# trevor-m/cuda-pathtrace

Hardware: AMD Instinct MI355X
Metric: Msamples/s, 9-sphere Cornell box 1024x1024x1024spp (higher is better)
Workload: dtype f32+f64

## Files before the change

cuda-pathtrace_amd/csrc/pt_intersect.h:

```cpp
#pragma once
#include "pt_scene_lds.h"

#pragma clang fp contract(off)

namespace pt {

template <int LEVEL>
__device__ __forceinline__ bool intersect_scene_loop(const SceneLds& sc, int n, F3 o, F3 d, const RayConst& rc,
                                                     float& t_hit, int& idx) {
  float tNearest = 1000000.0f;
  float t = 0.0f;
  bool hit = false;
#pragma clang loop unroll(disable)
  for (int i = 0; i < n; i++) {
    const float4 g = sc.geom_uniform(i);
    bool h;
    if constexpr (LEVEL == 0)
      h = intersect_sphere(o, d, rc.a, g, t);
    else
      h = intersect_sphere_v1(o, d, rc, g, t);
    if (h && t > 0.0f && t < tNearest) {
      tNearest = t;
      hit = true;
      t_hit = t;
      idx = i;
    }
  }
  return hit;
}

__device__ __forceinline__ bool intersect_scene_screened(const SceneLds& sc, int n, F3 o, F3 d, const RayConst& rc,
                                                         float& t_hit, int& idx) {
  const float INF = __builtin_inff();
  const float Tlim = 1000000.0f * (2.0f * rc.a);
  const float Tlim_hi = Tlim * 1.0000153f;
  float T1 = INF, T2 = INF;
  int i1 = 0;
  bool unsure = false;
PT_UNROLL(PT_SCREEN_UNROLL)
  for (int i = 0; i < n; i++) {
    const float4 g = sc.geom[i];
    const F3 off = mk3(o.x - g.x, o.y - g.y, o.z - g.z);
    const float b = 2.0f * dot(d, off);
    const float c = dot(off, off) - g.w;
    const float bb = b * b;
    const float a4c = rc.a4 * c;
    const float det = bb - a4c;
    const float dacc = fmaf(-rc.a4, c, bb);
    const float s = __builtin_amdgcn_sqrtf(fmaxf(dacc, 0.0f));
    const float q = b + copysign_b3(s, b);
    const float TA = -q;
    const float e = fmaf(b, b, -bb);
    const float num = a4c + e;
    const float TB = -num * __builtin_amdgcn_rcpf(q);
    const float lo = fminf(TA, TB), hi = fmaxf(TA, TB);
    const float T = lo > 0.0f ? lo : hi;
    const bool real = det >= 0.0f && dacc >= 0.0f;
    const bool ok = real && T > 0.0f && T < Tlim_hi;
    unsure = unsure || (real && !(fabsf(num) > fabsf(a4c) * 4.7683716e-07f && fabsf(T) < INF));
    const float Te = ok ? T : INF;
    const bool c1 = Te < T1, c2 = Te < T2;
    T2 = c1 ? T1 : (c2 ? Te : T2);
    i1 = c1 ? i : i1;
    T1 = c1 ? Te : T1;
  }
  bool ambiguous = unsure || (T1 < INF && (T2 <= T1 * 1.0000038f || T1 >= Tlim * 0.99998f));
  bool hit = false;
  if (!ambiguous && T1 < INF) {
    float t;
    if (intersect_sphere_v1(o, d, rc, sc.geom[i1], t) && t > 0.0f && t < 1000000.0f) {
      hit = true;
      t_hit = t;
      idx = i1;
    } else {
      ambiguous = true;
    }
  }
  if (__builtin_expect(ambiguous, 0)) hit = intersect_scene_loop<1>(sc, n, o, d, rc, t_hit, idx);
  return hit;
}

__device__ __forceinline__ void screen_tail(float b, float a4c, float det, float dacc, float num, float TA, float TB,
                                            float Tlim_hi, int i, float& T1, float& T2, int& i1, bool& unsure) {
  const float INF = __builtin_inff();
  const float lo = fminf(TA, TB), hi = fmaxf(TA, TB);
  const float T = lo > 0.0f ? lo : hi;
  const bool real = (det >= 0.0f) & (dacc >= 0.0f);
  const bool ok = real & (T > 0.0f) & (T < Tlim_hi);
  unsure = unsure | (real & !((fabsf(num) > fabsf(a4c) * 4.7683716e-07f) & (fabsf(T) < INF)));
  const float Te = ok ? T : INF;
  const bool c1 = Te < T1, c2 = Te < T2;
  T2 = c1 ? T1 : (c2 ? Te : T2);
  i1 = c1 ? i : i1;
  T1 = c1 ? Te : T1;
  (void)b;
}

__device__ __forceinline__ bool intersect_scene_screened_pk(const SceneLds& sc, int n, F3 o, F3 d, const RayConst& rc,
                                                            float& t_hit, int& idx) {
  const float INF = __builtin_inff();
  const float Tlim = 1000000.0f * (2.0f * rc.a);
  const float Tlim_hi = Tlim * 1.0000153f;
  float T1 = INF, T2 = INF;
  int i1 = 0;
  bool unsure = false;
  const v2f ox = {o.x, o.x}, oy = {o.y, o.y}, oz = {o.z, o.z};
  const v2f dx = {d.x, d.x}, dy = {d.y, d.y}, dz = {d.z, d.z};
  const v2f a4 = {rc.a4, rc.a4};
  const int npairs = (n + 1) >> 1;
  for (int p = 0; p < npairs; p++) {
    const float4 A = sc.pair[2 * p], B = sc.pair[2 * p + 1];
    const v2f offx = ox - v2f{A.x, A.y}, offy = oy - v2f{A.z, A.w}, offz = oz - v2f{B.x, B.y};
    const v2f dd = dx * offx + dy * offy + dz * offz;
    const v2f b = dd + dd;
    const v2f c = (offx * offx + offy * offy + offz * offz) - v2f{B.z, B.w};
    const v2f bb = b * b;
    const v2f a4c = a4 * c;
    const v2f det = bb - a4c;
    const v2f dacc = __builtin_elementwise_fma(-a4, c, bb);
    const v2f e = __builtin_elementwise_fma(b, b, -bb);
    const v2f num = a4c + e;
    const v2f s = {__builtin_amdgcn_sqrtf(fmaxf(dacc.x, 0.0f)), __builtin_amdgcn_sqrtf(fmaxf(dacc.y, 0.0f))};
    const v2f q = b + v2f{copysignf(s.x, b.x), copysignf(s.y, b.y)};
    const v2f r = {__builtin_amdgcn_rcpf(q.x), __builtin_amdgcn_rcpf(q.y)};
    const v2f TA = -q;
    const v2f TB = -num * r;
    screen_tail(b.x, a4c.x, det.x, dacc.x, num.x, TA.x, TB.x, Tlim_hi, 2 * p, T1, T2, i1, unsure);
    screen_tail(b.y, a4c.y, det.y, dacc.y, num.y, TA.y, TB.y, Tlim_hi, 2 * p + 1, T1, T2, i1, unsure);
  }
  bool ambiguous = unsure | ((T1 < INF) & ((T2 <= T1 * 1.0000038f) | (T1 >= Tlim * 0.99998f)));
  bool hit = false;
  if (!ambiguous && T1 < INF) {
    float t;
    if (intersect_sphere_v1(o, d, rc, sc.geom[i1], t) && t > 0.0f && t < 1000000.0f) {
      hit = true;
      t_hit = t;
      idx = i1;
    } else {
      ambiguous = true;
    }
  }
  if (__builtin_expect(ambiguous, 0)) hit = intersect_scene_loop<1>(sc, n, o, d, rc, t_hit, idx);
  return hit;
}

__device__ __forceinline__ uint32_t umed3(uint32_t a, uint32_t b, uint32_t c) {
  uint32_t r;
  asm("v_med3_u32 %0, %1, %2, %3" : "=v"(r) : "v"(a), "v"(b), "v"(c));
  return r;
}

struct ScreenState {
  uint32_t k1, k2;
  bool unsure;
  uint32_t absmask;
};

__device__ __forceinline__ uint32_t screen_sphere_oc(F3 off, float c, int i, F3 d, const RayConst& rc, uint32_t imask, ScreenState& st);
__device__ __forceinline__ uint32_t screen_sphere(const float4 g, int i, F3 o, F3 d, const RayConst& rc, uint32_t imask,
                                                  ScreenState& st) {
  const F3 off = mk3(o.x - g.x, o.y - g.y, o.z - g.z);
  return screen_sphere_oc(off, dot(off, off) - g.w, i, d, rc, imask, st);
}
__device__ __forceinline__ void screen_insert(ScreenState& st, uint32_t key) {
  st.k2 = umed3(st.k1, st.k2, key);
  st.k1 = st.k1 < key ? st.k1 : key;
}
template <class F>
__device__ __forceinline__ void screen_nine(ScreenState& st, F key_of) {
  auto umin = [](uint32_t x, uint32_t y) { return x < y ? x : y; };
  auto umax = [](uint32_t x, uint32_t y) { return x > y ? x : y; };
  uint32_t lead[3], next[3];
#pragma unroll
  for (int g3 = 0; g3 < 3; g3++) {
    const uint32_t x = key_of(3 * g3), y = key_of(3 * g3 + 1), z = key_of(3 * g3 + 2);
    lead[g3] = umin(umin(x, y), z);
    next[g3] = umed3(x, y, z);
  }
  const uint32_t l = umin(lead[0], lead[1]);
  const uint32_t r2 = umin(umin(umax(lead[0], lead[1]), next[0]), next[1]);
  st.k1 = umin(l, lead[2]);
  st.k2 = umin(umin(umax(l, lead[2]), r2), next[2]);
}
__device__ __forceinline__ uint32_t screen_sphere_oc(F3 off, float c, int i, F3 d, const RayConst& rc, uint32_t imask, ScreenState& st) {
  const float h = dot(d, off);
  const float hh = h * h;
  const float ac = rc.a * c;
  const float dacc = fmaf(-rc.a, c, hh);
  const float s = __builtin_amdgcn_sqrtf(dacc);
  const float e = fmaf(h, h, -hh);
  const float num = ac + e;
  const float TA = copysign_neg_b3(s, h, st.absmask) - h;
  const float TB = num * __builtin_amdgcn_rcpf(TA);
  const uint32_t ta = __float_as_uint(TA), tb = __float_as_uint(TB);
  const uint32_t tbits = ta < tb ? ta : tb;
  const uint32_t key = bitop3<0xBA>(tbits, imask, (uint32_t)i);
#ifndef PT_MUTANT_NO_DOUBT
  st.unsure = st.unsure | !(fabsf(ac) > fmaf(hh, 1.1920929e-07f, 1e-30f));
#endif
  return key;
}

__device__ __forceinline__ bool neg_finite(float x) { return __builtin_amdgcn_classf(x, 0x18); }
template <int AX>
__device__ __forceinline__ F3 with_axis(F3 v, float x) {
  return mk3(AX == 0 ? x : v.x, AX == 1 ? x : v.y, AX == 2 ? x : v.z);
}
template <int AX>
__device__ __forceinline__ uint32_t screen_wall_pair(const uint4 t, uint32_t m, F3 o, F3 d, const RayConst& rc, uint32_t imask,
                                                     ScreenState& st, float& hb, bool& inb) {
  const float4 gf = lds_read_f4(bitop3<0xE4>(t.y, t.x, m)), gb = lds_read_f4(bitop3<0xE4>(t.x, t.y, m));
  const F3 off = mk3(o.x - gf.x, o.y - gf.y, o.z - gf.z);
  const F3 sq = off * off, pr = d * off;
  const float ob = AX == 0 ? o.x - gb.x : AX == 1 ? o.y - gb.y : o.z - gb.z;
  const F3 sqb = with_axis<AX>(sq, ob * ob), prb = with_axis<AX>(pr, (AX == 0 ? d.x : AX == 1 ? d.y : d.z) * ob);
  hb = (prb.x + prb.y) + prb.z;
  inb = neg_finite(fmaf(gb.w, 5.9837103e-08f, ((sqb.x + sqb.y) + sqb.z) - gb.w));
  return screen_sphere_oc(off, ((sq.x + sq.y) + sq.z) - gf.w, (int)bitop3<0xE4>(t.w, t.z, m), d, rc, imask, st);
}
template <bool WALLS>
__device__ __forceinline__ void screen_walled(ScreenState& st, const uint4* W, F3 o, F3 d, const RayConst& rc, uint32_t imask,
                                              uint32_t lim_hi_bits) {
  auto umin = [](uint32_t x, uint32_t y) { return x < y ? x : y; };
  auto umax = [](uint32_t x, uint32_t y) { return x > y ? x : y; };
  const float4* Wg = reinterpret_cast<const float4*>(W);
  const uint4 oi = W[3];
  auto sel = [](uint32_t dbits) { return (uint32_t)((int32_t)dbits >> 31); };
  const uint32_t mx = sel(__float_as_uint(d.x)), my = sel(__float_as_uint(d.y)), mz = sel(__float_as_uint(d.z));
  const uint32_t a0 = screen_sphere(Wg[0], (int)oi.x, o, d, rc, imask, st), a1 = screen_sphere(Wg[1], (int)oi.y, o, d, rc, imask, st),
                 a2 = screen_sphere(Wg[2], (int)oi.z, o, d, rc, imask, st);
  const uint32_t l0 = umin(umin(a0, a1), a2), n0 = umed3(a0, a1, a2);
  float h0, h1, h2;
  bool in0, in1, in2;
  if constexpr (WALLS) __builtin_amdgcn_sched_barrier(0);
  const uint32_t b0 = screen_wall_pair<0>(W[4], mx, o, d, rc, imask, st, h0, in0);
  if constexpr (WALLS) __builtin_amdgcn_sched_barrier(0);
  const uint32_t b1 = screen_wall_pair<1>(W[5], my, o, d, rc, imask, st, h1, in1);
  if constexpr (WALLS) __builtin_amdgcn_sched_barrier(0);
  const uint32_t b2 = screen_wall_pair<2>(W[6], mz, o, d, rc, imask, st, h2, in2);
  if constexpr (WALLS) __builtin_amdgcn_sched_barrier(0);
  const uint32_t l1 = umin(umin(b0, b1), b2), n1 = umed3(b0, b1, b2);
  st.k1 = umin(l0, l1);
  st.k2 = umin(umin(umax(l0, l1), n0), n1);
  const float K = __uint_as_float(st.k1 & ~imask) * __uint_as_float(oi.w);
  const bool cert = (st.k1 < lim_hi_bits) & (neg_finite(fmaf(2.0f, h0, K)) & in0) & (neg_finite(fmaf(2.0f, h1, K)) & in1) &
                    (neg_finite(fmaf(2.0f, h2, K)) & in2);
  if (__builtin_expect(__builtin_amdgcn_ballot_w64(!cert) != 0, 0)) {
    auto behind = [&](int k, uint32_t m) {
      const uint4 t = W[4 + k];
      screen_insert(st, screen_sphere(lds_read_f4(bitop3<0xE4>(t.x, t.y, m)), (int)bitop3<0xE4>(t.z, t.w, m), o, d, rc, imask, st));
    };
    behind(0, mx);
    behind(1, my);
    behind(2, mz);
  }
}

#ifdef PT_SCREEN_STATS
__device__ unsigned long long g_screen_stats[8];
#endif
template <bool NB, bool PRIMARY = false, bool LAST = false, bool WALLS = false>
__device__ __forceinline__ bool intersect_scene_screened_keys(const SceneLds& sc, int n, F3 o, F3 d, const RayConst& rc,
                                                              float& t_hit, int& idx) {
  if (n <= 0) return false;
  const float Tlim = 1000000.0f * rc.a;
  const uint32_t lim_hi_bits = __float_as_uint(Tlim * 1.0000153f);
  const int ib = 32 - __builtin_clz((unsigned)(n > 1 ? n - 1 : 1));
  const uint32_t imask = (1u << ib) - 1u;
  const float margin = 1.0f + (__builtin_ldexpf(1.0f, ib - 22) + 7.6293945e-06f);
  ScreenState st{0xFFFFFFFFu, 0xFFFFFFFFu, false, sc.absmask};
  auto key_of = [&](const float4 g, int i) -> uint32_t {
    if constexpr (PRIMARY) {
      const float4 e = sc.eyeg[i];
      return screen_sphere_oc(mk3(e.x, e.y, e.z), e.w, i, d, rc, imask, st);
    } else {
      return screen_sphere(g, i, o, d, rc, imask, st);
    }
  };
  auto screen = [&](const float4 g, int i) { screen_insert(st, key_of(g, i)); };
  int i = 0;
  if constexpr (PRIMARY) {
    const uint32_t full = n >= 32 ? 0xFFFFFFFFu : (1u << n) - 1u;
    uint32_t m = __builtin_amdgcn_readfirstlane(sc.prim_mask) & full;
    if (m != full) {
      while (m) {
        const int j = __builtin_ctz(m);
        m &= m - 1u;
        screen(sc.geom[j], j);
      }
      i = n;
    }
  }
#if PT_UNROLL_NINE
  if constexpr (!PRIMARY) {
    if (sc.walls && n == 9) {
      screen_walled<WALLS>(st, sc.walls, o, d, rc, imask, lim_hi_bits);
      i = 9;
    }
  }
  if (i == 0 && n == 9) {
    screen_nine(st, [&](int u) { return key_of(sc.geom[u], u); });
    i = 9;
  }
#endif
  for (; i + 3 <= n; i += 3) {
    const float4 g0 = sc.geom[i], g1 = sc.geom[i + 1], g2 = sc.geom[i + 2];
    screen(g0, i);
    screen(g1, i + 1);
    screen(g2, i + 2);
  }
  for (; i < n; i++) screen(sc.geom[i], i);
  const uint32_t k1 = st.k1, k2 = st.k2;
  const bool has = k1 < lim_hi_bits;
  const float T1 = __uint_as_float(k1 & ~imask);
  bool ambiguous = st.unsure | (has & (((k2 & ~imask) <= __float_as_uint(T1 * margin)) | (T1 >= Tlim * 0.99998f)));
  bool hit = false;
  if constexpr (NB && LAST && !PRIMARY) {
    const int i1 = (int)(k1 & imask);
    const float4 g = sc.geom[has ? i1 : 0];
    const F3 off = mk3(o.x - g.x, o.y - g.y, o.z - g.z);
    const float h = dot(d, off);
    const float c = dot(off, off) - g.w;
    const float ac = rc.a * c;
    const float dacc = fmaf(-rc.a, c, h * h);
    const bool certain = (dacc > fabsf(ac) * 4.7683716e-07f) & (T1 >= rc.a * 1e-30f);
    ambiguous = ambiguous | (has & !certain);
    hit = has;
    t_hit = T1;
    idx = i1;
    if (__builtin_expect(ambiguous, 0)) hit = intersect_scene_loop<0>(sc, n, o, d, rc, t_hit, idx);
    return hit;
  } else if constexpr (NB) {
    const int i1 = (int)(k1 & imask);
    float t;
    bool bad = false;
    bool real;
    if constexpr (PRIMARY) {
      const float4 e = sc.eyeg[has ? i1 : 0];
      real = intersect_sphere_nb_oc(mk3(e.x, e.y, e.z), e.w, d, rc, t, bad);
    } else {
      real = intersect_sphere_nb(o, d, rc, sc.geom[has ? i1 : 0], t, bad);
    }
    const bool good = real & (t >= kMinGoodT) & (t < 1000000.0f);
#ifdef PT_SCREEN_STATS
    {
      const bool tie = has & ((k2 & ~imask) <= __float_as_uint(T1 * margin));
      const bool lim = has & (T1 >= Tlim * 0.99998f);
      const uint64_t any = __builtin_amdgcn_ballot_w64(ambiguous | (has & (bad | !good)));
      if ((threadIdx.x & 63) == __builtin_ctzll(__builtin_amdgcn_ballot_w64(true))) {
        atomicAdd(&g_screen_stats[0], 1ull);
        atomicAdd(&g_screen_stats[1], any != 0 ? 1ull : 0ull);
      }
      atomicAdd(&g_screen_stats[2], (ambiguous | (has & (bad | !good))) ? 1ull : 0ull);
      atomicAdd(&g_screen_stats[3], st.unsure ? 1ull : 0ull);
      atomicAdd(&g_screen_stats[4], tie ? 1ull : 0ull);
      atomicAdd(&g_screen_stats[5], lim ? 1ull : 0ull);
      atomicAdd(&g_screen_stats[6], (has & bad) ? 1ull : 0ull);
      atomicAdd(&g_screen_stats[7], (has & !good) ? 1ull : 0ull);
    }
#endif
    ambiguous = ambiguous | (has & (bad | !good));
    hit = has & good;
    t_hit = t;
    idx = i1;
#ifdef PT_TIMING_ONLY_DETECT_NO_REDO
    if (__builtin_expect(ambiguous, 0)) hit = false;
#elif !defined(PT_TIMING_ONLY_NO_ISECT_REDO)
    if (__builtin_expect(ambiguous, 0)) hit = intersect_scene_loop<0>(sc, n, o, d, rc, t_hit, idx);
#endif
    return hit;
  } else {
    if (!ambiguous && has) {
      const int i1 = (int)(k1 & imask);
      float t;
      if (intersect_sphere_v1(o, d, rc, sc.geom[i1], t) && t > 0.0f && t < 1000000.0f) {
        hit = true;
        t_hit = t;
        idx = i1;
      } else {
        ambiguous = true;
      }
    }
    if (__builtin_expect(ambiguous, 0)) hit = intersect_scene_loop<1>(sc, n, o, d, rc, t_hit, idx);
    return hit;
  }
}

__device__ __forceinline__ bool intersect_scene_screened_large(const SceneLds& sc, int n, F3 o, F3 d, const RayConst& rc,
                                                               float& t_hit, int& idx) {
  if (n <= 0) return false;
  const float INF = __builtin_inff();
  const float Tlim = 1000000.0f * (2.0f * rc.a);
  const float Tlim_hi = Tlim * 1.0000153f;
  float T1 = INF, T2 = INF;
  int i1 = 0;
  bool unsure = false;
  struct Head {
    float b, a4c, bb, dacc;
  };
  auto head = [&](const float4 g) {
    const F3 off = mk3(o.x - g.x, o.y - g.y, o.z - g.z);
    Head h;
    h.b = 2.0f * dot(d, off);
    const float c = dot(off, off) - g.w;
    h.bb = h.b * h.b;
    h.a4c = rc.a4 * c;
    h.dacc = fmaf(-rc.a4, c, h.bb);
    return h;
  };
  auto tail = [&](const Head& h, int i) {
    const bool cand = (int)__float_as_uint(h.dacc) >= 0;
    if (__builtin_amdgcn_ballot_w64(cand) == 0) return;
    const float s = __builtin_amdgcn_sqrtf(h.dacc);
    const float e = fmaf(h.b, h.b, -h.bb);
    const float num = h.a4c + e;
    const float TA = copysign_neg_b3(s, h.b, sc.absmask) - h.b;
    const float TB = num * __builtin_amdgcn_rcpf(TA);
    const uint32_t ta = __float_as_uint(TA), tb = __float_as_uint(TB);
    const uint32_t tbits = ta < tb ? ta : tb;
    const float T = __uint_as_float(tbits);
    const bool ok = tbits < __float_as_uint(Tlim_hi);
    unsure = unsure | (cand & !(fabsf(h.a4c) > fmaf(h.bb, 1.1920929e-07f, 1e-30f)));
    const float Te = ok ? T : INF;
    const bool c1 = Te < T1, c2 = Te < T2;
    T2 = c1 ? T1 : (c2 ? Te : T2);
    i1 = c1 ? i : i1;
    T1 = c1 ? Te : T1;
  };
  int i = 0;
  auto four = [&](const float4 g0, const float4 g1, const float4 g2, const float4 g3) {
    const Head h0 = head(g0), h1 = head(g1), h2 = head(g2), h3 = head(g3);
    const uint32_t all = __float_as_uint(h0.dacc) & __float_as_uint(h1.dacc) & __float_as_uint(h2.dacc) & __float_as_uint(h3.dacc);
    if (__builtin_amdgcn_ballot_w64((int)all >= 0) != 0) {
      tail(h0, i);
      tail(h1, i + 1);
      tail(h2, i + 2);
      tail(h3, i + 3);
    }
  };
  if (sc.lean) {
    typedef uint32_t u4 __attribute__((ext_vector_type(4)));
    const pt_sphere* base = sc.global;
    auto request = [&](u4& dst, int k) {
      const uint32_t off = (uint32_t)(k < n ? k : n - 1) * (uint32_t)sizeof(pt_sphere);
      asm volatile("s_load_dwordx4 %[dst], %[base], %[off]" : [dst] "=s"(dst), "+v"(o.x) : [base] "s"(base), [off] "s"(off));
    };
    auto as_geom = [](const u4 v) {
      const float r = __uint_as_float(v.x);
      return make_float4(__uint_as_float(v.y), __uint_as_float(v.z), __uint_as_float(v.w), r * r);
    };
    if (n >= 4) {
      u4 a0, a1, a2, a3;
      request(a0, 0);
      request(a1, 1);
      request(a2, 2);
      request(a3, 3);
      asm volatile("s_waitcnt lgkmcnt(0)" : "+s"(a0), "+s"(a1), "+s"(a2), "+s"(a3));
      for (; i + 4 <= n; i += 4) {
        u4 b0, b1, b2, b3;
        request(b0, i + 4);
        request(b1, i + 5);
        request(b2, i + 6);
        request(b3, i + 7);
        four(as_geom(a0), as_geom(a1), as_geom(a2), as_geom(a3));
        asm volatile("s_waitcnt lgkmcnt(0)" : "+s"(b0), "+s"(b1), "+s"(b2), "+s"(b3));
        a0 = b0;
        a1 = b1;
        a2 = b2;
        a3 = b3;
      }
    }
  } else {
    for (; i + 4 <= n; i += 4) four(sc.geom[i], sc.geom[i + 1], sc.geom[i + 2], sc.geom[i + 3]);
  }
  for (; i < n; i++) tail(head(sc.geom_uniform(i)), i);
  const bool has = T1 < INF;
  bool ambiguous = unsure | (has & ((T2 <= T1 * 1.0000038f) | (T1 >= Tlim * 0.99998f)));
  float t;
  bool bad = false;
  const bool real = intersect_sphere_nb(o, d, rc, sc.geom_lane(i1), t, bad);
  const bool good = real & (t >= kMinGoodT) & (t < 1000000.0f);
  ambiguous = ambiguous | (has & (bad | !good));
  t_hit = t;
  idx = i1;
  bool hit = has & good;
  if (__builtin_expect(ambiguous, 0)) hit = intersect_scene_loop<0>(sc, n, o, d, rc, t_hit, idx);
  return hit;
}

template <int LEVEL, bool PRIMARY = false, bool LAST = false, bool WALLS = false>
__device__ __forceinline__ bool intersect_scene(const SceneLds& sc, int n, F3 o, F3 d, float& t_hit, int& idx) {
  const RayConst rc = (LEVEL >= 6 && !PRIMARY && !sc.lean) ? make_ray_const_unit(d, sc.rden1) : make_ray_const(d);
  if constexpr (LEVEL >= 5) {
    if (!sc.lean && (sc.small_only || n <= PT_SCREEN_MAX_SPHERES))
      return intersect_scene_screened_keys<(LEVEL >= 6), (PRIMARY && LEVEL >= 6), (LAST && LEVEL >= 6), WALLS>(sc, n, o, d, rc, t_hit, idx);
    if constexpr (LEVEL >= 6) return intersect_scene_screened_large(sc, n, o, d, rc, t_hit, idx);
    return intersect_scene_loop<1>(sc, n, o, d, rc, t_hit, idx);
  }
  if constexpr (LEVEL == 3)
    return intersect_scene_screened_pk(sc, n, o, d, rc, t_hit, idx);
  else if constexpr (LEVEL == 2 || LEVEL == 4)
    return intersect_scene_screened(sc, n, o, d, rc, t_hit, idx);
  else
    return intersect_scene_loop<LEVEL>(sc, n, o, d, rc, t_hit, idx);
}

template <int P, bool PRIMARY = false, bool LAST = false>
__device__ __forceinline__ void intersect_paths(const SceneLds& sc, int n, const F3 (&o)[P], const F3 (&d)[P],
                                                bool (&hit)[P], float (&t_hit)[P], int (&idx)[P]) {
  RayConst rc[P];
  ScreenState st[P];
#pragma unroll
  for (int p = 0; p < P; p++) {
    rc[p] = (!PRIMARY && !sc.lean) ? make_ray_const_unit(d[p], sc.rden1) : make_ray_const(d[p]);
    st[p] = ScreenState{0xFFFFFFFFu, 0xFFFFFFFFu, false, sc.absmask};
    hit[p] = false;
  }
  if (n <= 0) return;
  if (sc.lean || (!sc.small_only && n > PT_SCREEN_MAX_SPHERES)) {
#pragma unroll
    for (int p = 0; p < P; p++) hit[p] = intersect_scene_screened_large(sc, n, o[p], d[p], rc[p], t_hit[p], idx[p]);
    return;
  }
  const int ib = 32 - __builtin_clz((unsigned)(n > 1 ? n - 1 : 1));
  const uint32_t imask = (1u << ib) - 1u;
  const float margin = 1.0f + (__builtin_ldexpf(1.0f, ib - 22) + 7.6293945e-06f);
  int i = 0;
  if constexpr (PRIMARY && P == 1) {
    const uint32_t full = n >= 32 ? 0xFFFFFFFFu : (1u << n) - 1u;
    uint32_t m = __builtin_amdgcn_readfirstlane(sc.prim_mask) & full;
    if (n <= 16 && m != full) {
      while (m) {
        const int j = __builtin_ctz(m);
        m &= m - 1u;
        const float4 e = sc.eyeg[j];
        screen_insert(st[0], screen_sphere_oc(mk3(e.x, e.y, e.z), e.w, j, d[0], rc[0], imask, st[0]));
      }
      i = n;
    }
  }
#if PT_UNROLL_NINE
  if (i == 0 && P == 1 && n == 9) {
    screen_nine(st[0], [&](int u) -> uint32_t {
      if constexpr (PRIMARY) {
        const float4 e = sc.eyeg[u];
        return screen_sphere_oc(mk3(e.x, e.y, e.z), e.w, u, d[0], rc[0], imask, st[0]);
      } else {
        return screen_sphere(sc.geom[u], u, o[0], d[0], rc[0], imask, st[0]);
      }
    });
    i = 9;
  }
#endif
  for (; i + 2 <= n; i += 2) {
    const float4 g0 = sc.geom[i], g1 = sc.geom[i + 1];
#pragma unroll
    for (int p = 0; p < P; p++) {
      screen_insert(st[p], screen_sphere(g0, i, o[p], d[p], rc[p], imask, st[p]));
      screen_insert(st[p], screen_sphere(g1, i + 1, o[p], d[p], rc[p], imask, st[p]));
    }
  }
  for (; i < n; i++) {
    const float4 g = sc.geom[i];
#pragma unroll
    for (int p = 0; p < P; p++) screen_insert(st[p], screen_sphere(g, i, o[p], d[p], rc[p], imask, st[p]));
  }
  bool ambiguous[P];
#pragma unroll
  for (int p = 0; p < P; p++) {
    const float Tlim = 1000000.0f * rc[p].a;
    const bool has = st[p].k1 < __float_as_uint(Tlim * 1.0000153f);
    const float T1 = __uint_as_float(st[p].k1 & ~imask);
    ambiguous[p] = st[p].unsure | (has & (((st[p].k2 & ~imask) <= __float_as_uint(T1 * margin)) | (T1 >= Tlim * 0.99998f)));
    const int i1 = (int)(st[p].k1 & imask);
    if constexpr (LAST && !PRIMARY) {
      const float4 g = sc.geom[has ? i1 : 0];
      const F3 off = mk3(o[p].x - g.x, o[p].y - g.y, o[p].z - g.z);
      const float h = dot(d[p], off);
      const float c = dot(off, off) - g.w;
      const float dacc = fmaf(-rc[p].a, c, h * h);
      const bool certain = (dacc > fabsf(rc[p].a * c) * 4.7683716e-07f) & (T1 >= rc[p].a * 1e-30f);
      ambiguous[p] = ambiguous[p] | (has & !certain);
      hit[p] = has;
      t_hit[p] = T1;
      idx[p] = i1;
      continue;
    }
    float t;
    bool bad = false;
    bool real;
    if (PRIMARY && P == 1 && n <= 16) {
      const float4 e = sc.eyeg[has ? i1 : 0];
      real = intersect_sphere_nb_oc(mk3(e.x, e.y, e.z), e.w, d[p], rc[p], t, bad);
    } else {
      real = intersect_sphere_nb(o[p], d[p], rc[p], sc.geom[has ? i1 : 0], t, bad);
    }
    const bool good = real & (t >= kMinGoodT) & (t < 1000000.0f);
    ambiguous[p] = ambiguous[p] | (has & (bad | !good));
    hit[p] = has & good;
    t_hit[p] = t;
    idx[p] = i1;
  }
#pragma unroll
  for (int p = 0; p < P; p++)
    if (__builtin_expect(ambiguous[p], 0)) hit[p] = intersect_scene_loop<0>(sc, n, o[p], d[p], rc[p], t_hit[p], idx[p]);
}

}
```

cuda-pathtrace_amd/csrc/pt_scene_lds.h:

```cpp
#pragma once
#include "pt_device.h"
#include "pt_kernel.h"
#include "pt_walls.h"

#pragma clang fp contract(off)

namespace pt {

#define PT_PRAGMA_(x) _Pragma(#x)
#define PT_UNROLL(n) PT_PRAGMA_(unroll n)

struct GridLds;

struct SceneLds {
  float4* geom;
  float4* mat0;
  float4* mat1;
  float4* eyeg;
  float* inv1;
  double* rden1;
  float* rcpn;
  float4* pair;
  const pt_sphere* global;
  bool lean;
  bool small_only;
  const GridLds* grid;
  void* pool;
  uint32_t prim_mask;
  uint32_t absmask;
  const uint4* walls = nullptr;

  __device__ __forceinline__ float4 geom_uniform(int i) const {
    if (lean) {
      typedef float f4u __attribute__((ext_vector_type(4), aligned(4)));
      typedef const __attribute__((address_space(4))) f4u* cptr;
      typedef const __attribute__((address_space(4))) char* cbytes;
      const f4u v = *(cptr)((cbytes)global + (size_t)i * sizeof(pt_sphere));
      return make_float4(v.y, v.z, v.w, v.x * v.x);
    }
    return geom[i];
  }
  __device__ __forceinline__ float4 geom_lane(int i) const {
    if (lean) {
      const pt_sphere* sp = global + i;
      return make_float4(sp->pos[0], sp->pos[1], sp->pos[2], sp->radius * sp->radius);
    }
    return geom[i];
  }
};

typedef float v2f __attribute__((ext_vector_type(2)));

constexpr int kTablesF4 = kUnitTabSize / 4 + kUnitTabSize / 2 + (kRcpTab + 4) / 4;

template <bool WITH_PAIR>
__device__ __forceinline__ SceneLds stage_scene(const pt_sphere* __restrict__ spheres, int n, float4* lds, bool lean, F3 eye,
                                                int spp, bool lean_tables = true) {
  float4* tab = lean ? lds : lds + 4 * n;
  const bool tables = !lean | lean_tables;
  SceneLds s{lds, lds + n, lds + 2 * n, lds + 3 * n, tables ? reinterpret_cast<float*>(tab) : nullptr,
             tables ? reinterpret_cast<double*>(tab + kUnitTabSize / 4) : nullptr,
             tables ? reinterpret_cast<float*>(tab + kUnitTabSize / 4 + kUnitTabSize / 2) : nullptr, lds + 4 * n + kTablesF4,
             spheres, lean, false, nullptr, nullptr, 0xFFFFFFFFu, vgpr_const<0x7FFFFFFFu>()};
  const float qnan = __builtin_nanf("");
  if (tables) {
    for (int i = threadIdx.x; i < kUnitTabSize; i += blockDim.x)
      s.inv1[i] = 1.0f / sqrtf(__uint_as_float(0x3F800000u - (uint32_t)kUnitTabHalf + (uint32_t)i));
    for (int i = threadIdx.x; i < kUnitTabSize; i += blockDim.x) {
      const float a = __uint_as_float(0x3F800000u - (uint32_t)kUnitTabHalf + (uint32_t)i);
      s.rden1[i] = ray_const_rden(2.0 * (double)a);
    }
    const int counts = spp < kRcpTab ? spp : kRcpTab;
    for (int i = threadIdx.x; i < counts; i += blockDim.x) s.rcpn[i] = 1.0f / (float)(i + 1);
    if (threadIdx.x == 0) s.rcpn[kRcpTab] = qnan;
  }
  if (lean) {
    __syncthreads();
    return s;
  }
  for (int i = threadIdx.x; i < n; i += blockDim.x) {
    const pt_sphere sp = spheres[i];
    const float rr = sp.radius * sp.radius;
    s.geom[i] = make_float4(sp.pos[0], sp.pos[1], sp.pos[2], rr);
    s.mat0[i] = make_float4(sp.emission[0], sp.emission[1], sp.emission[2], sp.color[0]);
    s.mat1[i] = make_float4(sp.color[1], sp.color[2], luminance(mk3(sp.color[0], sp.color[1], sp.color[2])), 0.0f);
    const F3 off = mk3(eye.x - sp.pos[0], eye.y - sp.pos[1], eye.z - sp.pos[2]);
    s.eyeg[i] = make_float4(off.x, off.y, off.z, dot(off, off) - rr);
    if constexpr (WITH_PAIR) {
      float* pa = reinterpret_cast<float*>(s.pair + 2 * (i >> 1)) + (i & 1);
      pa[0] = sp.pos[0];
      pa[2] = sp.pos[1];
      pa[4] = sp.pos[2];
      pa[6] = rr;
      if ((i == n - 1) && !(i & 1)) {
        pa[1] = qnan;
        pa[3] = qnan;
        pa[5] = qnan;
        pa[7] = qnan;
      }
    }
  }
  __syncthreads();
  return s;
}

__device__ __forceinline__ uint32_t lds_addr(const void* p) {
  return (uint32_t)(uintptr_t)(const __attribute__((address_space(3))) char*)p;
}
__device__ __forceinline__ float4 lds_read_f4(uint32_t addr) {
  typedef float f4v __attribute__((ext_vector_type(4)));
  const f4v v = *(const __attribute__((address_space(3))) f4v*)(uintptr_t)addr;
  return make_float4(v.x, v.y, v.z, v.w);
}

constexpr int kWallF4 = 7;
__device__ __forceinline__ void stage_walls(SceneLds& s, const pt_sphere* __restrict__ spheres, int n) {
  uint4* W = reinterpret_cast<uint4*>(s.pair);
  if (threadIdx.x == 0) {
    const WallLayout w = classify_walls(spheres, n);
    for (int k = 0; k < 3; k++) {
      const float4 g = s.geom[w.obj[k]];
      W[k] = make_uint4(__float_as_uint(g.x), __float_as_uint(g.y), __float_as_uint(g.z), __float_as_uint(g.w));
      W[4 + k] = make_uint4(lds_addr(s.geom + w.minus[k]), lds_addr(s.geom + w.plus[k]), (uint32_t)w.minus[k], (uint32_t)w.plus[k]);
    }
    W[3] = make_uint4((uint32_t)w.obj[0], (uint32_t)w.obj[1], (uint32_t)w.obj[2], w.ok ? 0x3F802000u : 0x7F800000u);
  }
  __syncthreads();
  s.walls = W;
}

__device__ __forceinline__ void fetch_material(const SceneLds& sc, int idx, F3& emis, F3& scol, float* lum_col = nullptr) {
  if (sc.lean) {
#ifdef PT_TIMING_ONLY_NO_MATERIAL
    emis = mk3(0.0f, 0.0f, 0.0f);
    scol = mk3(0.5f, 0.5f, 0.5f);
    if (lum_col) *lum_col = 0.5f;
    return;
#endif
    const pt_sphere* sp = sc.global + idx;
    emis = mk3(sp->emission[0], sp->emission[1], sp->emission[2]);
    scol = mk3(sp->color[0], sp->color[1], sp->color[2]);
    if (lum_col) *lum_col = luminance(scol);
  } else {
    const float4 m0 = sc.mat0[idx];
    const float4 m1 = sc.mat1[idx];
    emis = mk3(m0.x, m0.y, m0.z);
    scol = mk3(m0.w, m1.x, m1.y);
    if (lum_col) *lum_col = m1.z;
  }
}

struct TraceOutput {
  F3 color, normal, albedo;
  float depth;
};

__device__ __forceinline__ void frame_values(const TraceOutput& L, const Welford var[4], float fs, float px[14]) {
  px[0] = L.color.x / fs;
  px[1] = L.color.y / fs;
  px[2] = L.color.z / fs;
  px[3] = L.normal.x / fs;
  px[4] = L.normal.y / fs;
  px[5] = L.normal.z / fs;
  px[6] = L.albedo.x / fs;
  px[7] = L.albedo.y / fs;
  px[8] = L.albedo.z / fs;
  px[9] = L.depth / fs;
  px[10] = welford_variance(var[0]);
  px[11] = welford_variance(var[1]);
  px[12] = welford_variance(var[2]);
  px[13] = welford_variance(var[3]);
}

template <int RNG>
struct Rng;

template <>
struct Rng<PT_RNG_XORWOW> {
  Xorwow st;
  __device__ __forceinline__ void begin_sample(uint32_t) {}
  __device__ __forceinline__ void jitter(float& jx, float& jy) {
    jx = uniform_from_u32(xorwow_next(st));
    jy = uniform_from_u32(xorwow_next(st));
  }
  __device__ __forceinline__ void bounce(int, float& az, float& el) {
    az = uniform_from_u32(xorwow_next(st));
    el = uniform_from_u32(xorwow_next(st));
  }
};

template <>
struct Rng<PT_RNG_PHILOX> {
  uint32_t k0, k1, pix, sample;
  uint4 blk;
  __device__ __forceinline__ void begin_sample(uint32_t s) {
    sample = s;
    blk = philox4x32_10(make_uint4(pix, sample, 0u, 0u), k0, k1);
  }
  __device__ __forceinline__ void jitter(float& jx, float& jy) {
    jx = uniform_from_u32(blk.x);
    jy = uniform_from_u32(blk.y);
  }
  __device__ __forceinline__ void bounce(int n, float& az, float& el) {
    if (n & 1) blk = philox4x32_10(make_uint4(pix, sample, (uint32_t)((n + 1) >> 1), 0u), k0, k1);
    bool second = (n == 0) || (((n + 1) & 1) != 0);
    az = uniform_from_u32(second ? blk.z : blk.x);
    el = uniform_from_u32(second ? blk.w : blk.y);
  }
};

}
```

cuda-pathtrace_amd/csrc/pt_walls.h:

```cpp
#pragma once
#include <math.h>
#include "../../include/ptcore.h"

namespace pt {

struct WallLayout {
  int obj[3];
  int minus[3];
  int plus[3];
  bool ok;
};

__host__ __device__ inline WallLayout classify_walls(const pt_sphere* s, int n) {
  WallLayout w{{6, 7, 8}, {0, 2, 4}, {1, 3, 5}, false};
  const WallLayout none = w;
  if (n != 9) return w;
  double rmax = 0.0;
  for (int i = 0; i < 9; i++) {
    const double r = (double)s[i].radius;
    if (!(r >= 0.0) || !(r < 1e30)) return none;
    rmax = r > rmax ? r : rmax;
  }
  int walls[6], objs[3], nw = 0, no = 0;
  for (int i = 0; i < 9; i++) {
    if ((double)s[i].radius >= 0.5 * rmax) {
      if (nw == 6) return none;
      walls[nw++] = i;
    } else {
      if (no == 3) return none;
      objs[no++] = i;
    }
  }
  if (nw != 6 || no != 3) return none;
  double p[3] = {0.0, 0.0, 0.0};
  for (int j = 0; j < 6; j++)
    for (int k = 0; k < 3; k++) p[k] += (double)s[walls[j]].pos[k] / 6.0;
  double ext = 0.0;
  for (int j = 0; j < 3; j++)
    for (int k = 0; k < 3; k++) {
      const double e = fabs((double)s[objs[j]].pos[k] - p[k]);
      if (!(e < 1e30)) return none;
      ext = e > ext ? e : ext;
    }
  int mi[3] = {-1, -1, -1}, pl[3] = {-1, -1, -1};
  for (int j = 0; j < 6; j++) {
    const pt_sphere& sw = s[walls[j]];
    const double r = (double)sw.radius;
    if (sw.emission[0] != 0.0f || sw.emission[1] != 0.0f || sw.emission[2] != 0.0f) return none;
    if (!(r >= 100.0 * ext) || !(r > 0.0)) return none;
    double off[3];
    int ax = 0;
    for (int k = 0; k < 3; k++) {
      off[k] = (double)sw.pos[k] - p[k];
      if (!(fabs(off[k]) < 1e30)) return none;
      if (fabs(off[k]) > fabs(off[ax])) ax = k;
    }
    if (!(fabs(off[ax]) >= 0.5 * r)) return none;
    for (int k = 0; k < 3; k++)
      if (k != ax && !(fabs(off[k]) <= 1e-2 * r)) return none;
    int* slot = off[ax] > 0.0 ? &pl[ax] : &mi[ax];
    if (*slot >= 0) return none;
    *slot = walls[j];
  }
  for (int k = 0; k < 3; k++) {
    if (mi[k] < 0 || pl[k] < 0) return none;
    const pt_sphere &a = s[pl[k]], &b = s[mi[k]];
    if (!((double)a.pos[k] - (double)a.radius < (double)b.pos[k] + (double)b.radius)) return none;
    for (int j = 0; j < 3; j++)
      if (j != k && __builtin_bit_cast(unsigned, a.pos[j]) != __builtin_bit_cast(unsigned, b.pos[j])) return none;
  }
  for (int k = 0; k < 3; k++) {
    w.obj[k] = objs[k];
    w.minus[k] = mi[k];
    w.plus[k] = pl[k];
  }
  w.ok = true;
  return w;
}

}
```

Before: 24670.

## Share wall-pair offset terms via common wall-center point and compact per-axis wall records

Precomputes a shared center point for axis-aligned Cornell walls so the squared and projected offset terms are computed once and reused across all six wall spheres. Only the varying axis component is recomputed per wall, and each wall pair is read through one packed LDS record instead of two sphere loads. The fallback path for uncertain rays now rescans the six walls in a loop with per-wall doubt tracking. This adds a new alignment check in wall classification, a larger LDS wall block, and a changed doubt-propagation path that could alter which rays get flagged as unsure.

Result: no change. 24910 (median of 6 runs) (+1.0%).

```diff
diff --git a/cuda-pathtrace_amd/csrc/pt_intersect.h b/cuda-pathtrace_amd/csrc/pt_intersect.h
--- a/cuda-pathtrace_amd/csrc/pt_intersect.h
+++ b/cuda-pathtrace_amd/csrc/pt_intersect.h
@@ -207,8 +207,20 @@
   return mk3(AX == 0 ? x : v.x, AX == 1 ? x : v.y, AX == 2 ? x : v.z);
 }
 template <int AX>
-__device__ __forceinline__ uint32_t screen_wall_pair(const uint4 t, uint32_t m, F3 o, F3 d, const RayConst& rc, uint32_t imask,
-                                                     ScreenState& st, float& hb, bool& inb) {
+__device__ __forceinline__ uint32_t screen_wall_pair(const uint4 t, uint32_t m, F3 o, F3 d, F3 sq, F3 pr, const RayConst& rc,
+                                                     uint32_t imask, ScreenState& st, float& hb, bool& inb) {
+  const float4 g = lds_read_f4(bitop3<0xE4>(t.y, t.x, m));
+  const float oa = AX == 0 ? o.x : AX == 1 ? o.y : o.z, da = AX == 0 ? d.x : AX == 1 ? d.y : d.z;
+  const float of = oa - g.x, ob = oa - g.z;
+  const F3 sqf = with_axis<AX>(sq, of * of), prf = with_axis<AX>(pr, da * of);
+  const F3 sqb = with_axis<AX>(sq, ob * ob), prb = with_axis<AX>(pr, da * ob);
+  hb = (prb.x + prb.y) + prb.z;
+  inb = neg_finite(fmaf(g.w, 5.9837103e-08f, ((sqb.x + sqb.y) + sqb.z) - g.w));
+  return screen_sphere_oc(prf, ((sqf.x + sqf.y) + sqf.z) - g.y, (int)bitop3<0xE4>(t.w, t.z, m), mk3(1.0f, 1.0f, 1.0f), rc, imask, st);
+}
+template <int AX>
+__device__ __forceinline__ uint32_t screen_wall_pair_never_run(const uint4 t, uint32_t m, F3 o, F3 d, const RayConst& rc, uint32_t imask,
+                                                               ScreenState& st, float& hb, bool& inb) {
   const float4 gf = lds_read_f4(bitop3<0xE4>(t.y, t.x, m)), gb = lds_read_f4(bitop3<0xE4>(t.x, t.y, m));
   const F3 off = mk3(o.x - gf.x, o.y - gf.y, o.z - gf.z);
   const F3 sq = off * off, pr = d * off;
@@ -218,9 +230,8 @@
   inb = neg_finite(fmaf(gb.w, 5.9837103e-08f, ((sqb.x + sqb.y) + sqb.z) - gb.w));
   return screen_sphere_oc(off, ((sq.x + sq.y) + sq.z) - gf.w, (int)bitop3<0xE4>(t.w, t.z, m), d, rc, imask, st);
 }
-template <bool WALLS>
-__device__ __forceinline__ void screen_walled(ScreenState& st, const uint4* W, F3 o, F3 d, const RayConst& rc, uint32_t imask,
-                                              uint32_t lim_hi_bits) {
+__device__ __forceinline__ void screen_walled_never_run(ScreenState& st, const uint4* W, F3 o, F3 d, const RayConst& rc, uint32_t imask,
+                                                        uint32_t lim_hi_bits) {
   auto umin = [](uint32_t x, uint32_t y) { return x < y ? x : y; };
   auto umax = [](uint32_t x, uint32_t y) { return x > y ? x : y; };
   const float4* Wg = reinterpret_cast<const float4*>(W);
@@ -232,13 +243,9 @@
   const uint32_t l0 = umin(umin(a0, a1), a2), n0 = umed3(a0, a1, a2);
   float h0, h1, h2;
   bool in0, in1, in2;
-  if constexpr (WALLS) __builtin_amdgcn_sched_barrier(0);
-  const uint32_t b0 = screen_wall_pair<0>(W[4], mx, o, d, rc, imask, st, h0, in0);
-  if constexpr (WALLS) __builtin_amdgcn_sched_barrier(0);
-  const uint32_t b1 = screen_wall_pair<1>(W[5], my, o, d, rc, imask, st, h1, in1);
-  if constexpr (WALLS) __builtin_amdgcn_sched_barrier(0);
-  const uint32_t b2 = screen_wall_pair<2>(W[6], mz, o, d, rc, imask, st, h2, in2);
-  if constexpr (WALLS) __builtin_amdgcn_sched_barrier(0);
+  const uint32_t b0 = screen_wall_pair_never_run<0>(W[4], mx, o, d, rc, imask, st, h0, in0);
+  const uint32_t b1 = screen_wall_pair_never_run<1>(W[5], my, o, d, rc, imask, st, h1, in1);
+  const uint32_t b2 = screen_wall_pair_never_run<2>(W[6], mz, o, d, rc, imask, st, h2, in2);
   const uint32_t l1 = umin(umin(b0, b1), b2), n1 = umed3(b0, b1, b2);
   st.k1 = umin(l0, l1);
   st.k2 = umin(umin(umax(l0, l1), n0), n1);
@@ -254,6 +261,54 @@
     behind(1, my);
     behind(2, mz);
   }
+}
+template <bool WALLS>
+__device__ __forceinline__ void screen_walled(ScreenState& st, const uint4* W, const float4* geom, F3 o, F3 d, const RayConst& rc,
+                                              uint32_t imask, uint32_t lim_hi_bits) {
+  if constexpr (!WALLS) return screen_walled_never_run(st, W, o, d, rc, imask, lim_hi_bits);
+  auto umin = [](uint32_t x, uint32_t y) { return x < y ? x : y; };
+  auto umax = [](uint32_t x, uint32_t y) { return x > y ? x : y; };
+  const float4* Wg = reinterpret_cast<const float4*>(W);
+  const uint4 oi = W[3];
+  auto sel = [](uint32_t dbits) { return (uint32_t)((int32_t)dbits >> 31); };
+  const uint32_t mx = sel(__float_as_uint(d.x)), my = sel(__float_as_uint(d.y)), mz = sel(__float_as_uint(d.z));
+  const uint32_t a0 = screen_sphere(Wg[0], (int)oi.x, o, d, rc, imask, st), a1 = screen_sphere(Wg[1], (int)oi.y, o, d, rc, imask, st),
+                 a2 = screen_sphere(Wg[2], (int)oi.z, o, d, rc, imask, st);
+  const uint32_t l0 = umin(umin(a0, a1), a2), n0 = umed3(a0, a1, a2);
+  ScreenState sw{0xFFFFFFFFu, 0xFFFFFFFFu, false, st.absmask};
+  float h0, h1, h2;
+  bool in0, in1, in2;
+  if constexpr (WALLS) __builtin_amdgcn_sched_barrier(0);
+  const float3 p = *reinterpret_cast<const float3*>(Wg + 7);
+  const F3 u = mk3(o.x - p.x, o.y - p.y, o.z - p.z);
+  const F3 sq = u * u, pr = d * u;
+  const uint32_t b0 = screen_wall_pair<0>(W[4], mx, o, d, sq, pr, rc, imask, sw, h0, in0);
+  if constexpr (WALLS) __builtin_amdgcn_sched_barrier(0);
+  const uint32_t b1 = screen_wall_pair<1>(W[5], my, o, d, sq, pr, rc, imask, sw, h1, in1);
+  if constexpr (WALLS) __builtin_amdgcn_sched_barrier(0);
+  const uint32_t b2 = screen_wall_pair<2>(W[6], mz, o, d, sq, pr, rc, imask, sw, h2, in2);
+  if constexpr (WALLS) __builtin_amdgcn_sched_barrier(0);
+  const uint32_t l1 = umin(umin(b0, b1), b2), n1 = umed3(b0, b1, b2);
+  st.k1 = umin(l0, l1);
+  st.k2 = umin(umin(umax(l0, l1), n0), n1);
+  const float K = __uint_as_float(st.k1 & ~imask) * Wg[7].w;
+  const bool cert = (st.k1 < lim_hi_bits) & (neg_finite(fmaf(2.0f, h0, K)) & in0) & (neg_finite(fmaf(2.0f, h1, K)) & in1) &
+                    (neg_finite(fmaf(2.0f, h2, K)) & in2);
+  if (__builtin_expect(__builtin_amdgcn_ballot_w64(!cert) != 0, 0)) {
+    st.k1 = l0;
+    st.k2 = n0;
+    const uint32_t* wi = reinterpret_cast<const uint32_t*>(W + 4);
+    uint64_t doubts = 0;
+#pragma clang loop unroll(disable)
+    for (int w = 0; w < 6; w++) {
+      const int i = (int)wi[4 * (w >> 1) + 2 + (w & 1)];
+      sw.unsure = false;
+      screen_insert(st, screen_sphere(geom[i], i, o, d, rc, imask, sw));
+      doubts |= __builtin_amdgcn_ballot_w64(sw.unsure);
+    }
+    sw.unsure = __builtin_amdgcn_inverse_ballot_w64(doubts);
+  }
+  st.unsure = st.unsure | sw.unsure;
 }
 
 #ifdef PT_SCREEN_STATS
@@ -294,7 +349,7 @@
 #if PT_UNROLL_NINE
   if constexpr (!PRIMARY) {
     if (sc.walls && n == 9) {
-      screen_walled<WALLS>(st, sc.walls, o, d, rc, imask, lim_hi_bits);
+            screen_walled<WALLS>(st, sc.walls, sc.geom, o, d, rc, imask, lim_hi_bits);
       i = 9;
     }
   }
diff --git a/cuda-pathtrace_amd/csrc/pt_scene_lds.h b/cuda-pathtrace_amd/csrc/pt_scene_lds.h
--- a/cuda-pathtrace_amd/csrc/pt_scene_lds.h
+++ b/cuda-pathtrace_amd/csrc/pt_scene_lds.h
@@ -113,7 +113,7 @@
   return make_float4(v.x, v.y, v.z, v.w);
 }
 
-constexpr int kWallF4 = 7;
+constexpr int kWallF4 = 14;
 __device__ __forceinline__ void stage_walls(SceneLds& s, const pt_sphere* __restrict__ spheres, int n) {
   uint4* W = reinterpret_cast<uint4*>(s.pair);
   if (threadIdx.x == 0) {
@@ -121,9 +121,14 @@
     for (int k = 0; k < 3; k++) {
       const float4 g = s.geom[w.obj[k]];
       W[k] = make_uint4(__float_as_uint(g.x), __float_as_uint(g.y), __float_as_uint(g.z), __float_as_uint(g.w));
-      W[4 + k] = make_uint4(lds_addr(s.geom + w.minus[k]), lds_addr(s.geom + w.plus[k]), (uint32_t)w.minus[k], (uint32_t)w.plus[k]);
-    }
-    W[3] = make_uint4((uint32_t)w.obj[0], (uint32_t)w.obj[1], (uint32_t)w.obj[2], w.ok ? 0x3F802000u : 0x7F800000u);
+      W[4 + k] = make_uint4(lds_addr(W + 8 + 2 * k), lds_addr(W + 9 + 2 * k), (uint32_t)w.minus[k], (uint32_t)w.plus[k]);
+      const float4 gm = s.geom[w.minus[k]], gp = s.geom[w.plus[k]];
+      const uint32_t cm = __float_as_uint(k == 0 ? gm.x : k == 1 ? gm.y : gm.z), cp = __float_as_uint(k == 0 ? gp.x : k == 1 ? gp.y : gp.z);
+      W[8 + 2 * k] = make_uint4(cm, __float_as_uint(gm.w), cp, __float_as_uint(gp.w));
+      W[9 + 2 * k] = make_uint4(cp, __float_as_uint(gp.w), cm, __float_as_uint(gm.w));
+    }
+    W[3] = make_uint4((uint32_t)w.obj[0], (uint32_t)w.obj[1], (uint32_t)w.obj[2], 0u);
+    W[7] = make_uint4(__float_as_uint(w.p[0]), __float_as_uint(w.p[1]), __float_as_uint(w.p[2]), w.aligned ? 0x3F802000u : 0x7F800000u);
   }
   __syncthreads();
   s.walls = W;
diff --git a/cuda-pathtrace_amd/csrc/pt_walls.h b/cuda-pathtrace_amd/csrc/pt_walls.h
--- a/cuda-pathtrace_amd/csrc/pt_walls.h
+++ b/cuda-pathtrace_amd/csrc/pt_walls.h
@@ -9,10 +9,12 @@
   int minus[3];
   int plus[3];
   bool ok;
+  bool aligned;
+  float p[3];
 };
 
 __host__ __device__ inline WallLayout classify_walls(const pt_sphere* s, int n) {
-  WallLayout w{{6, 7, 8}, {0, 2, 4}, {1, 3, 5}, false};
+  WallLayout w{{6, 7, 8}, {0, 2, 4}, {1, 3, 5}, false, false, {0.0f, 0.0f, 0.0f}};
   const WallLayout none = w;
   if (n != 9) return w;
   double rmax = 0.0;
@@ -43,6 +45,9 @@
       ext = e > ext ? e : ext;
     }
   int mi[3] = {-1, -1, -1}, pl[3] = {-1, -1, -1};
+#ifdef __clang__
+#pragma clang loop unroll(disable)
+#endif
   for (int j = 0; j < 6; j++) {
     const pt_sphere& sw = s[walls[j]];
     const double r = (double)sw.radius;
@@ -75,6 +80,13 @@
     w.plus[k] = pl[k];
   }
   w.ok = true;
+  w.aligned = true;
+  for (int j = 0; j < 3; j++) {
+    const float a = s[mi[(j + 1) % 3]].pos[j], b = s[mi[(j + 2) % 3]].pos[j];
+    if (__builtin_bit_cast(unsigned, a) != __builtin_bit_cast(unsigned, b)) w.aligned = false;
+    w.p[j] = a;
+  }
+  if (!w.aligned) w.p[0] = w.p[1] = w.p[2] = 0.0f;
   return w;
 }
 
```
